# Lakonik/MVEdit

Measured on AMD Instinct MI355X. Metric: multi-view denoise-steps/sec (32 views, 512^2), higher is better.
Workload: dtype f16; 1 GPU; 32-view 512x512 get_noise_pred: 64 SD-1.5 UNet forwards (64x64 latents, ctx 77x768) + CFG per step; ControlNet residuals zero; views=32, latent=64, cfg=True, parallelism=views/1

## Files before the change

mvedit_amd/csrc/attention.hip:

```cpp
#include "common.h"

#include <stdlib.h>
#include <type_traits>

namespace {

constexpr int NT = 256;

struct AttnParams {
    const void* Q; const void* K; const void* V; const void* K2; const void* V2; void* O;
    int ldq, ldk, ldv, ldk2, ldv2, ldo;
    int B, Lq, Lk, Lk2, heads;
    float scale_log2e;
    int prescaled;
    const int* skip_if;
};

template <int DP, bool KSW2> __device__ __forceinline__ int k_perm(int row, int pc) {
    if constexpr (DP == 64) return pc ^ ((row >> 1) & 7);
    else if constexpr (KSW2) return pc ^ (((row >> 3) & 1) << 1);
    else return pc ^ ((row >> 2) & 3);
}
template <int DP, bool KSW2> __device__ __forceinline__ int k_swz(int row, int chunk) {
    return row * (DP * 2) + (k_perm<DP, KSW2>(row, chunk) << 4);
}

typedef __attribute__((address_space(3))) void* lds_ptr_t;
typedef const __attribute__((address_space(1))) void* gbl_ptr_t;
typedef float f32x8 __attribute__((ext_vector_type(8)));

__device__ __attribute__((aligned(16))) unsigned int g_attn_zero_page[4] = {0u, 0u, 0u, 0u};

template <int KB2, bool VSW2> __device__ __forceinline__ int v_swz2(int row, int chunk) {
    if constexpr (KB2 == 128) return row * 256 + ((chunk ^ (row & 15) ^ (VSW2 ? (row >> 3) & 7 : 0)) << 4);
    else return row * 128 + ((chunk ^ ((row >> 1) & 7) ^ (VSW2 ? (row >> 4) & 7 : 0)) << 4);
}

template <class Tag, int D, bool SEG2, int QF = 2, int KB2X = 0, int OCC = 0, bool KSW2 = false, bool VSW2 = false>
__global__ __launch_bounds__(NT, (OCC ? OCC : (D > 80 ? 1 : 2))) void k_attention2(const AttnParams p) {
    constexpr int QB = 64 * QF;
    constexpr int DP = (D + 31) / 32 * 32;
    constexpr int KS = DP / 32;
    constexpr int DC = D / 8;
    constexpr int DVF = (D + 15) / 16;
    constexpr int KB2 = KB2X ? KB2X : (D > 64 ? 64 : 128);
    constexpr int NH = KB2 / 64;
    constexpr int CPR = DP / 8;
    constexpr int KROW = DP * 2;
    constexpr int VROW = KB2 * 2;
    constexpr int K_BYTES = KB2 * KROW;
    constexpr int V_BYTES = DVF * 16 * VROW;
    constexpr int K_INSTR = K_BYTES / 1024 / 4;
    static_assert((K_BYTES / 1024) % 4 == 0, "K tile must split evenly over 4 waves");
    constexpr int V_TASKS = (KB2 / 2) * DC;
    constexpr int V_PER_T = (V_TASKS + NT - 1) / NT;
    constexpr bool ONES = (D % 16) != 0;
    constexpr int L_G = (D % 16) / 4, L_R = (D % 16) % 4;
    typedef typename Tag::V8 V8;
    typedef typename Tag::T T;

    __shared__ __attribute__((aligned(16))) unsigned char smem[2 * K_BYTES + 2 * V_BYTES];
    unsigned char* Kbuf = smem;
    unsigned char* Vbuf = smem + 2 * K_BYTES;

    const int tid = threadIdx.x, lane = tid & 63, wid = tid >> 6;
    const int g = lane >> 4, l16 = lane & 15;

    const int q_tiles = (p.Lq + QB - 1) / QB;
    const unsigned nblk = (unsigned)(q_tiles * p.heads * p.B);
    const unsigned bid = p.skip_if ? mve_xcd_remap_halves(blockIdx.x, nblk, nblk / 2) : mve_xcd_remap(blockIdx.x, nblk);
    const int qt = bid % q_tiles;
    const int h = (bid / q_tiles) % p.heads;
    const int b = bid / (q_tiles * p.heads);
    if (mve_second_half_skipped(p.skip_if, 2 * b >= p.B)) return;
    const int Ltot = p.Lk + p.Lk2;

    const T* Qp = reinterpret_cast<const T*>(p.Q);
    const T* zero = reinterpret_cast<const T*>(g_attn_zero_page);
    const T* kb1 = reinterpret_cast<const T*>(p.K) + (size_t)b * p.Lk * p.ldk + h * D;
    const T* vb1 = reinterpret_cast<const T*>(p.V) + (size_t)b * p.Lk * p.ldv + h * D;
    const T* kb2 = SEG2 ? reinterpret_cast<const T*>(p.K2) + (size_t)b * p.Lk2 * p.ldk2 + h * D : nullptr;
    const T* vb2 = SEG2 ? reinterpret_cast<const T*>(p.V2) + (size_t)b * p.Lk2 * p.ldv2 + h * D : nullptr;
    auto k_row = [&](int j) -> const T* {
        if constexpr (SEG2) { if (j >= p.Lk) return kb2 + (size_t)(j - p.Lk) * p.ldk2; }
        return kb1 + (size_t)j * p.ldk;
    };
    auto v_row = [&](int j) -> const T* {
        if constexpr (SEG2) { if (j >= p.Lk) return vb2 + (size_t)(j - p.Lk) * p.ldv2; }
        return vb1 + (size_t)j * p.ldv;
    };

    for (int i = tid; i < 2 * V_BYTES / 16; i += NT) reinterpret_cast<u32x4*>(Vbuf)[i] = u32x4{0u, 0u, 0u, 0u};
    __syncthreads();
    if constexpr (ONES) {
        const unsigned short one = __builtin_bit_cast(unsigned short, Tag::from_f32(1.0f));
        const unsigned two = (unsigned)one | ((unsigned)one << 16);
        for (int i = tid; i < 2 * (VROW / 4); i += NT) {
            const int buf = i / (VROW / 4), wofs = i - buf * (VROW / 4);
            *reinterpret_cast<unsigned*>(Vbuf + buf * V_BYTES + D * VROW + wofs * 4) = two;
        }
    }

    V8 qf[QF][KS];
    const int q_base = qt * QB + wid * (16 * QF);
#pragma unroll
    for (int f = 0; f < QF; ++f) {
        int q = q_base + f * 16 + l16;
        q = q < p.Lq ? q : p.Lq - 1;
        const T* row = Qp + ((size_t)b * p.Lq + q) * p.ldq + h * D;
#pragma unroll
        for (int ks = 0; ks < KS; ++ks) {
            const int c = ks * 4 + g;
            u32x4 v = {0u, 0u, 0u, 0u};
            if (c < DC) v = *reinterpret_cast<const u32x4*>(row + c * 8);
            qf[f][ks] = __builtin_bit_cast(V8, v);
        }
    }

    int kd_row[K_INSTR], kd_col[K_INSTR];
#pragma unroll
    for (int i = 0; i < K_INSTR; ++i) {
        const int pos = (wid * K_INSTR + i) * 64 + lane;
        const int row = pos / CPR, pc = pos - row * CPR;
        const int c = k_perm<DP, KSW2>(row, pc);
        kd_row[i] = row;
        kd_col[i] = c < DC ? c * 8 : -1;
    }
    int vt_key[V_PER_T], vt_col[V_PER_T], vt_lds[V_PER_T];
#pragma unroll
    for (int i = 0; i < V_PER_T; ++i) {
        const int task = tid + i * NT;
        const int pair = task / DC, c = task - pair * DC;
        const int key = 2 * pair;
        const int kk = key >> 5, hh = (key >> 4) & 1, gg = (key >> 2) & 3, jj = key & 3;
        const int pos = 32 * kk + 8 * gg + 4 * hh + jj;
        vt_key[i] = task < V_TASKS ? key : -1;
        vt_col[i] = c * 8;
        vt_lds[i] = ((pos >> 3) << 16) | ((pos & 7) * 2);
    }
    int koff[KS];
#pragma unroll
    for (int ks = 0; ks < KS; ++ks) koff[ks] = k_swz<DP, KSW2>(l16, ks * 4 + g);
    constexpr bool VTAB = VSW2 && DVF * NH * 2 <= 12;
    int voff[VTAB ? 1 : NH * 2], voff2[VTAB ? DVF : 1][NH * 2];
    if constexpr (VTAB) {
#pragma unroll
        for (int i = 0; i < DVF; ++i)
#pragma unroll
            for (int s2 = 0; s2 < NH * 2; ++s2) voff2[i][s2] = v_swz2<KB2, true>(i * 16 + l16, s2 * 4 + g);
    } else {
#pragma unroll
        for (int s2 = 0; s2 < NH * 2; ++s2) voff[s2] = v_swz2<KB2, VSW2>(l16, s2 * 4 + g);
    }
    auto vx = [](int i) { return !VSW2 ? 0 : (KB2 == 128 ? ((2 * i) & 7) << 4 : (i & 7) << 4); };

    auto dma_k = [&](int t, int buf) {
        const int j0 = t * KB2;
#pragma unroll
        for (int i = 0; i < K_INSTR; ++i) {
            int j = j0 + kd_row[i];
            j = j < Ltot ? j : Ltot - 1;
            const T* src = kd_col[i] >= 0 ? k_row(j) + kd_col[i] : zero;
            __builtin_amdgcn_global_load_lds((gbl_ptr_t)src, (lds_ptr_t)(Kbuf + buf * K_BYTES + (wid * K_INSTR + i) * 1024), 16, 0, 0);
        }
    };
    u32x4 vreg[V_PER_T][2];
    auto load_v = [&](int t) {
        const int j0 = t * KB2;
#pragma unroll
        for (int i = 0; i < V_PER_T; ++i) {
            if (vt_key[i] >= 0) {
                int j = j0 + vt_key[i];
                const int ja = j < Ltot ? j : Ltot - 1, jb = j + 1 < Ltot ? j + 1 : Ltot - 1;
                vreg[i][0] = *reinterpret_cast<const u32x4*>(v_row(ja) + vt_col[i]);
                vreg[i][1] = *reinterpret_cast<const u32x4*>(v_row(jb) + vt_col[i]);
            }
        }
    };
    auto store_v = [&](int buf) {
        unsigned char* Vs = Vbuf + buf * V_BYTES;
#pragma unroll
        for (int i = 0; i < V_PER_T; ++i) {
            if (vt_key[i] >= 0) {
                const int chunk = vt_lds[i] >> 16, within = vt_lds[i] & 0xffff;
                const unsigned short* a = reinterpret_cast<const unsigned short*>(&vreg[i][0]);
                const unsigned short* bb = reinterpret_cast<const unsigned short*>(&vreg[i][1]);
#pragma unroll
                for (int e = 0; e < 8; ++e)
                    *reinterpret_cast<unsigned*>(Vs + v_swz2<KB2, VSW2>(vt_col[i] + e, chunk) + within) = (unsigned)a[e] | ((unsigned)bb[e] << 16);
            }
        }
    };

    f32x4 oacc[DVF][QF];
#pragma unroll
    for (int i = 0; i < DVF; ++i)
#pragma unroll
        for (int f = 0; f < QF; ++f) oacc[i][f] = f32x4{0.f, 0.f, 0.f, 0.f};
    float m_run[QF], l_run[QF];
#pragma unroll
    for (int f = 0; f < QF; ++f) { m_run[f] = -INFINITY; l_run[f] = 0.f; }

    auto do_half = [&](const unsigned char* Ks, const unsigned char* Vs, int hf, int key0, auto masked_tag) {
        constexpr bool MASKED = decltype(masked_tag)::value;
        f32x4 s[4][QF];
#pragma unroll
        for (int kf = 0; kf < 4; ++kf)
#pragma unroll
            for (int f = 0; f < QF; ++f) s[kf][f] = f32x4{0.f, 0.f, 0.f, 0.f};
#pragma unroll
        for (int ks = 0; ks < KS; ++ks) {
#pragma unroll
            for (int kf = 0; kf < 4; ++kf) {
                const V8 ka = *reinterpret_cast<const V8*>(Ks + koff[ks] + (hf * 64 + kf * 16) * KROW);
#pragma unroll
                for (int f = 0; f < QF; ++f) s[kf][f] = Tag::mfma16(ka, qf[f][ks], s[kf][f]);
            }
        }
        if constexpr (MASKED) {
#pragma unroll
            for (int kf = 0; kf < 4; ++kf)
#pragma unroll
                for (int r = 0; r < 4; ++r)
                    if (key0 + kf * 16 + g * 4 + r >= Ltot) {
#pragma unroll
                        for (int f = 0; f < QF; ++f) s[kf][f][r] = -INFINITY;
                    }
        }
        V8 pf[QF][2];
#pragma unroll
        for (int f = 0; f < QF; ++f) {
            float mx = -INFINITY;
#pragma unroll
            for (int kf = 0; kf < 4; ++kf)
#pragma unroll
                for (int r = 0; r < 4; ++r) mx = fmaxf(mx, s[kf][f][r]);
            mx = mve_max_xor32(mve_max_xor16(mx));
            const float mxs = mx * p.scale_log2e;
            if (__any(mxs > m_run[f])) {
                const float m_new = fmaxf(m_run[f], mxs);
                const float alpha = __builtin_amdgcn_exp2f(m_run[f] - m_new);
                m_run[f] = m_new;
                if constexpr (!ONES) l_run[f] *= alpha;
#pragma unroll
                for (int i = 0; i < DVF; ++i)
#pragma unroll
                    for (int r = 0; r < 4; ++r) oacc[i][f][r] *= alpha;
            }
            const float mr = m_run[f];
            float psum = 0.f;
#pragma unroll
            for (int kk = 0; kk < 2; ++kk) {
                f32x8 e;
                {
                    typedef float f32x2 __attribute__((ext_vector_type(2)));
                    const f32x2 sc2 = {p.scale_log2e, p.scale_log2e}, mr2 = {mr, mr};
                    const f32x4 a4 = s[2 * kk][f], b4 = s[2 * kk + 1][f];
                    const f32x2 t0 = __builtin_elementwise_fma(f32x2{a4[0], a4[1]}, sc2, -mr2);
                    const f32x2 t1 = __builtin_elementwise_fma(f32x2{a4[2], a4[3]}, sc2, -mr2);
                    const f32x2 t2 = __builtin_elementwise_fma(f32x2{b4[0], b4[1]}, sc2, -mr2);
                    const f32x2 t3 = __builtin_elementwise_fma(f32x2{b4[2], b4[3]}, sc2, -mr2);
                    e[0] = __builtin_amdgcn_exp2f(t0[0]); e[1] = __builtin_amdgcn_exp2f(t0[1]);
                    e[2] = __builtin_amdgcn_exp2f(t1[0]); e[3] = __builtin_amdgcn_exp2f(t1[1]);
                    e[4] = __builtin_amdgcn_exp2f(t2[0]); e[5] = __builtin_amdgcn_exp2f(t2[1]);
                    e[6] = __builtin_amdgcn_exp2f(t3[0]); e[7] = __builtin_amdgcn_exp2f(t3[1]);
                }
                if constexpr (!ONES) {
#pragma unroll
                    for (int r = 0; r < 8; ++r) psum += e[r];
                }
                pf[f][kk] = __builtin_convertvector(e, V8);
            }
            if constexpr (!ONES) l_run[f] += psum;
        }
#pragma unroll
        for (int kk = 0; kk < 2; ++kk) {
#pragma unroll
            for (int i = 0; i < DVF; ++i) {
                V8 va;
                if constexpr (VTAB) va = *reinterpret_cast<const V8*>(Vs + voff2[i][hf * 2 + kk]);
                else {
                    int a = voff[hf * 2 + kk];
                    if constexpr (VSW2) { if (vx(i)) asm volatile("v_xor_b32 %0, %1, %0" : "+v"(a) : "s"(vx(i))); }
                    va = *reinterpret_cast<const V8*>(Vs + a + i * 16 * VROW);
                }
#pragma unroll
                for (int f = 0; f < QF; ++f) oacc[i][f] = Tag::mfma16(va, pf[f][kk], oacc[i][f]);
            }
        }
    };

    const int n_tiles = (Ltot + KB2 - 1) / KB2;
    dma_k(0, 0);
    load_v(0);
    __syncthreads();
    store_v(0);
    __syncthreads();

    for (int t = 0; t < n_tiles; ++t) {
        const int cur = t & 1;
        if (t + 1 < n_tiles) { dma_k(t + 1, cur ^ 1); load_v(t + 1); }
        const unsigned char* Ks = Kbuf + cur * K_BYTES;
        const unsigned char* Vs = Vbuf + cur * V_BYTES;
#pragma unroll
        for (int hf = 0; hf < NH; ++hf) {
            const int key0 = t * KB2 + hf * 64;
            if (key0 + 64 <= Ltot) {
                do_half(Ks, Vs, hf, key0, std::false_type{});
            } else if (key0 < Ltot) {
                do_half(Ks, Vs, hf, key0, std::true_type{});
            }
        }
        if (t + 1 < n_tiles) store_v(cur ^ 1);
        __syncthreads();
    }

    typedef T T4 __attribute__((ext_vector_type(4)));
#pragma unroll
    for (int f = 0; f < QF; ++f) {
        float l;
        if constexpr (ONES) {
            l = __shfl(oacc[DVF - 1][f][L_R], L_G * 16 + l16, 64);
        } else {
            l = l_run[f];
            l += __shfl_xor(l, 16, 64);
            l += __shfl_xor(l, 32, 64);
        }
        const float inv = 1.0f / l;
        const int q = q_base + f * 16 + l16;
        if (q < p.Lq) {
            T* orow = reinterpret_cast<T*>(p.O) + ((size_t)b * p.Lq + q) * p.ldo + h * D;
#pragma unroll
            for (int i = 0; i < DVF; ++i) {
                const int dv = i * 16 + g * 4;
                if (dv < D) {
                    T4 pk;
#pragma unroll
                    for (int r = 0; r < 4; ++r) pk[r] = Tag::from_f32(oacc[i][f][r] * inv);
                    *reinterpret_cast<T4*>(orow + dv) = pk;
                }
            }
        }
    }
}

__device__ __attribute__((aligned(16))) unsigned short g_attn_ones_f16[8] = {0x3C00u, 0, 0, 0, 0, 0, 0, 0};
__device__ __attribute__((aligned(16))) unsigned short g_attn_ones_bf16[8] = {0x3F80u, 0, 0, 0, 0, 0, 0, 0};

__device__ unsigned long long g_attn_prof[4] = {0ull, 0ull, 0ull, 0ull};

typedef short s16x4 __attribute__((ext_vector_type(4)));
typedef short s16x8 __attribute__((ext_vector_type(8)));
typedef float f32x2 __attribute__((ext_vector_type(2)));

__device__ __forceinline__ void attn_dma16(const void* gsrc, unsigned lds_dst) {
    unsigned keep;
    asm volatile("s_mov_b32 %0, m0\n\ts_mov_b32 m0, %2\n\ts_nop 0\n\tglobal_load_lds_dwordx4 %1, off\n\ts_mov_b32 m0, %0"
                 : "=&s"(keep) : "v"(gsrc), "s"(lds_dst) : "memory");
}

template <class Tag, bool SEG2, int NW, int NST, int WPS, bool PRE, bool PIPE, int ABL = 0>
__global__ __launch_bounds__(64 * NW, WPS) void k_attention3(const AttnParams p) {
    constexpr int D = 40, KB = 64, QB = 32 * NW;
    constexpr int K_ROW = 80, V_ROW = 96;
    constexpr int K_BYTES = KB * K_ROW, V_BYTES = KB * V_ROW, STAGE = K_BYTES + V_BYTES;
    constexpr int N_DMA = STAGE / 1024, K_DMA = K_BYTES / 1024, DMA_PER_WAVE = (N_DMA + NW - 1) / NW;
    static_assert(STAGE % 1024 == 0 && K_BYTES % 1024 == 0, "stage must split into whole LDS-DMA instructions");
    static_assert(NST >= 2 && NST <= 4, "2 to 4 LDS stages");
    typedef typename Tag::V8 V8;
    typedef typename Tag::T T;
    typedef T T2 __attribute__((ext_vector_type(2)));
    typedef T T4 __attribute__((ext_vector_type(4)));

    __shared__ __attribute__((aligned(16))) unsigned char smem[NST * STAGE];

    const int tid = threadIdx.x, lane = tid & 63, wid = tid >> 6;
    const int l32 = lane & 31, hi = lane >> 5, l16 = lane & 15, g = lane >> 4;
    unsigned long long prof_t0 = 0, prof_r0 = 0;
    if constexpr ((ABL & 1024) != 0) asm volatile("s_memtime %0\n\ts_memrealtime %1\n\ts_waitcnt lgkmcnt(0)" : "=s"(prof_t0), "=s"(prof_r0) :: "memory");

    const int q_tiles = (p.Lq + QB - 1) / QB;
    const unsigned nblk = (unsigned)(q_tiles * p.heads * p.B);
    const unsigned bid = p.skip_if ? mve_xcd_remap_halves(blockIdx.x, nblk, nblk / 2) : mve_xcd_remap(blockIdx.x, nblk);
    const int qt = bid % q_tiles;
    const int h = (bid / q_tiles) % p.heads;
    const int b = bid / (q_tiles * p.heads);
    if (mve_second_half_skipped(p.skip_if, 2 * b >= p.B)) return;
    const int Ltot = p.Lk + p.Lk2;

    const T* kb1 = reinterpret_cast<const T*>(p.K) + (size_t)b * p.Lk * p.ldk + h * D;
    const T* vb1 = reinterpret_cast<const T*>(p.V) + (size_t)b * p.Lk * p.ldv + h * D;
    const T* kb2 = SEG2 ? reinterpret_cast<const T*>(p.K2) + (size_t)b * p.Lk2 * p.ldk2 + h * D : nullptr;
    const T* vb2 = SEG2 ? reinterpret_cast<const T*>(p.V2) + (size_t)b * p.Lk2 * p.ldv2 + h * D : nullptr;
    const T* ones = reinterpret_cast<const T*>(std::is_same<T, f16>::value ? g_attn_ones_f16 : g_attn_ones_bf16);
    auto k_row = [&](int j) -> const T* {
        if constexpr (SEG2) { if (j >= p.Lk) return kb2 + (size_t)(j - p.Lk) * p.ldk2; }
        return kb1 + (size_t)j * p.ldk;
    };
    auto v_row = [&](int j) -> const T* {
        if constexpr (SEG2) { if (j >= p.Lk) return vb2 + (size_t)(j - p.Lk) * p.ldv2; }
        return vb1 + (size_t)j * p.ldv;
    };

    const int q_base = qt * QB + wid * 32;
    V8 qf[3];
    {
        int q = q_base + l32;
        q = q < p.Lq ? q : p.Lq - 1;
        const T* row = reinterpret_cast<const T*>(p.Q) + ((size_t)b * p.Lq + q) * p.ldq + h * D;
        qf[0] = __builtin_bit_cast(V8, *reinterpret_cast<const u32x4*>(row + 8 * hi));
        qf[1] = __builtin_bit_cast(V8, *reinterpret_cast<const u32x4*>(row + 16 + 8 * hi));
        u32x4 t = {0u, 0u, 0u, 0u};
        if (hi == 0) t = *reinterpret_cast<const u32x4*>(row + 32);
        qf[2] = __builtin_bit_cast(V8, t);
    }

    const int wv = __builtin_amdgcn_readfirstlane(wid);
    const unsigned smem_base = (unsigned)(uintptr_t)(lds_ptr_t)smem;
    int d_key[DMA_PER_WAVE], d_col[DMA_PER_WAVE];
    const T* d_src[DMA_PER_WAVE];
    int d_ld[DMA_PER_WAVE];
#pragma unroll
    for (int i = 0; i < DMA_PER_WAVE; ++i) {
        const int inst = wv + NW * i;
        const int o = inst * 1024 + lane * 16;
        if (inst < K_DMA) {
            const int c = o >> 4;
            d_key[i] = c / 5; d_col[i] = (c - d_key[i] * 5) * 8;
            d_ld[i] = p.ldk;
            d_src[i] = kb1 + (size_t)d_key[i] * p.ldk + d_col[i];
        } else {
            const int c = (o - K_BYTES) >> 4;
            const int r = c / 6, col = c - r * 6;
            d_key[i] = (r & ~12) | ((r & 4) << 1) | ((r & 8) >> 1);
            d_col[i] = col < 5 ? col * 8 : -1;
            d_ld[i] = col < 5 ? p.ldv : 0;
            d_src[i] = col < 5 ? vb1 + (size_t)d_key[i] * p.ldv + d_col[i] : ones;
        }
    }
    auto dma_fast = [&](int stage_off) {
#pragma unroll
        for (int i = 0; i < DMA_PER_WAVE; ++i) {
            const int inst = wv + NW * i;
            if (inst < N_DMA) {
                attn_dma16(d_src[i], smem_base + stage_off + inst * 1024);
                d_src[i] += (size_t)KB * d_ld[i];
            }
        }
    };
    auto dma_any = [&](int t, int stage_off) {
        const int j0 = t * KB;
#pragma unroll
        for (int i = 0; i < DMA_PER_WAVE; ++i) {
            const int inst = wv + NW * i;
            if (inst < N_DMA) {
                int j = j0 + d_key[i];
                j = j < Ltot ? j : Ltot - 1;
                const T* src = inst < K_DMA ? k_row(j) + d_col[i] : (d_col[i] >= 0 ? v_row(j) + d_col[i] : ones);
                attn_dma16(src, smem_base + stage_off + inst * 1024);
            }
        }
    };
    const int n_tiles = (Ltot + KB - 1) / KB, n_full = Ltot / KB;
    auto dma = [&](int t, int stage_off) {
        if constexpr ((ABL & 4) != 0) return;
        if constexpr (SEG2) dma_any(t, stage_off);
        else { if (t < n_full) dma_fast(stage_off); else dma_any(t, stage_off); }
    };
    const int n_mine = (N_DMA - wv + NW - 1) / NW;

    const int k_off01 = l32 * K_ROW + hi * 16;
    const int k_off2 = l32 * K_ROW + 64;
    const int v_off = K_BYTES + (lane >> 2) * V_ROW + (lane & 3) * 8;

    f32x4 oacc[3][2];
#pragma unroll
    for (int i = 0; i < 3; ++i)
#pragma unroll
        for (int f = 0; f < 2; ++f) oacc[i][f] = f32x4{0.f, 0.f, 0.f, 0.f};
    float m_run = PRE ? 0.f : -INFINITY;
    const float sc = p.scale_log2e;

    f32x16 negm;
#pragma unroll
    for (int r = 0; r < 16; ++r) negm[r] = 0.f;

    struct S2 { f32x16 a, b; };
    struct PB { unsigned w[2][2][4]; };

    auto qk = [&](const unsigned char* St) -> S2 {
        f32x16 zero16;
#pragma unroll
        for (int r = 0; r < 16; ++r) zero16[r] = 0.f;
        S2 s;
#pragma unroll
        for (int st = 0; st < 3; ++st) {
            const int o = st < 2 ? k_off01 + 32 * st : k_off2;
            V8 ka, kb_;
            if constexpr ((ABL & 128) != 0) { ka = qf[st]; kb_ = qf[(st + 1) % 3]; }
            else { ka = *reinterpret_cast<const V8*>(St + o); kb_ = *reinterpret_cast<const V8*>(St + o + 32 * K_ROW); }
            if constexpr ((ABL & 32) != 0) {
                asm volatile("" :: "v"(ka), "v"(kb_));
                if (st == 0) { s.a = negm; s.b = negm; }
                continue;
            }
            if (PRE && st == 0) {
                if constexpr (std::is_same<T, f16>::value) {
                    asm volatile("v_mfma_f32_32x32x16_f16 %0, %1, %2, %3" : "=&v"(s.a) : "v"(ka), "v"(qf[0]), "v"(negm));
                    asm volatile("v_mfma_f32_32x32x16_f16 %0, %1, %2, %3" : "=&v"(s.b) : "v"(kb_), "v"(qf[0]), "v"(negm));
                } else {
                    asm volatile("v_mfma_f32_32x32x16_bf16 %0, %1, %2, %3" : "=&v"(s.a) : "v"(ka), "v"(qf[0]), "v"(negm));
                    asm volatile("v_mfma_f32_32x32x16_bf16 %0, %1, %2, %3" : "=&v"(s.b) : "v"(kb_), "v"(qf[0]), "v"(negm));
                }
            } else {
                s.a = Tag::mfma32(ka, qf[st], st == 0 ? zero16 : s.a);
                s.b = Tag::mfma32(kb_, qf[st], st == 0 ? zero16 : s.b);
            }
        }
        return s;
    };

    auto softmax_max = [&](S2& s, int key0, auto masked_tag, bool first) {
        constexpr bool MASKED = decltype(masked_tag)::value;
        if constexpr (MASKED) {
#pragma unroll
            for (int r = 0; r < 16; ++r) {
                if (key0 + (r & 3) + 8 * (r >> 2) + 4 * hi >= Ltot) s.a[r] = -INFINITY;
                if (key0 + 32 + (r & 3) + 8 * (r >> 2) + 4 * hi >= Ltot) s.b[r] = -INFINITY;
            }
        }
        float mx = fmaxf(s.a[0], s.b[0]);
        if constexpr ((ABL & 16) == 0) {
#pragma unroll
            for (int r = 1; r < 16; ++r) mx = fmaxf(fmaxf(mx, s.a[r]), s.b[r]);
            mx = mve_max_xor32(mx);
        }
        float a0 = 1.f, a1 = 1.f;
        bool rescale = false;
        if constexpr (PRE) {
            if (__builtin_expect(first || __any(mx > 0.f), 0)) {
                const float delta = first ? mx : fmaxf(mx, 0.f);
                m_run += delta;
#pragma unroll
                for (int r = 0; r < 16; ++r) { s.a[r] -= delta; s.b[r] -= delta; negm[r] = -m_run; }
                if (!first) {
                    const float alpha = __builtin_amdgcn_exp2f(-delta);
                    const auto ar = __builtin_amdgcn_permlane16_swap(__float_as_uint(alpha), __float_as_uint(alpha), false, false);
                    a0 = __uint_as_float(ar[0]); a1 = __uint_as_float(ar[1]);
                    rescale = true;
                }
            }
        } else {
            const float mxs = mx * sc;
            if (__builtin_expect(__any(mxs > m_run), 0)) {
                const float m_new = fmaxf(m_run, mxs);
                const float alpha = __builtin_amdgcn_exp2f(m_run - m_new);
                m_run = m_new;
                const auto ar = __builtin_amdgcn_permlane16_swap(__float_as_uint(alpha), __float_as_uint(alpha), false, false);
                a0 = __uint_as_float(ar[0]); a1 = __uint_as_float(ar[1]);
                rescale = true;
            }
        }
        if (rescale) {
#pragma unroll
            for (int i = 0; i < 3; ++i)
#pragma unroll
                for (int r = 0; r < 4; ++r) { oacc[i][0][r] *= a0; oacc[i][1][r] *= a1; }
        }
    };

    auto softmax_exp = [&](const S2& s) -> PB {
        const float nm = -m_run;
        PB pb;
#pragma unroll
        for (int kb = 0; kb < 2; ++kb) {
            const f32x16& sk = kb ? s.b : s.a;
            unsigned pk[8];
#pragma unroll
            for (int r2 = 0; r2 < 8; ++r2) {
                float e0, e1;
                if constexpr (PRE && (ABL & 8) != 0) {
                    e0 = sk[2 * r2]; e1 = sk[2 * r2 + 1];
                } else if constexpr (PRE) {
                    e0 = __builtin_amdgcn_exp2f(sk[2 * r2]);
                    e1 = __builtin_amdgcn_exp2f(sk[2 * r2 + 1]);
                } else {
                    e0 = __builtin_amdgcn_exp2f(__builtin_fmaf(sk[2 * r2], sc, nm));
                    e1 = __builtin_amdgcn_exp2f(__builtin_fmaf(sk[2 * r2 + 1], sc, nm));
                }
                pk[r2] = __builtin_bit_cast(unsigned, __builtin_convertvector(f32x2{e0, e1}, T2));
            }
#pragma unroll
            for (int v = 0; v < 4; ++v) {
                const int ai = v < 2 ? v : v + 2;
                if constexpr ((ABL & 512) != 0) { pb.w[kb][0][v] = pk[ai]; pb.w[kb][1][v] = pk[ai + 2]; continue; }
                const auto r = __builtin_amdgcn_permlane16_swap(pk[ai], pk[ai + 2], false, false);
                pb.w[kb][0][v] = r[0];
                pb.w[kb][1][v] = r[1];
            }
        }
        return pb;
    };

    auto pv = [&](const unsigned char* St, const PB& pb) {
#pragma unroll
        for (int kb = 0; kb < 2; ++kb) {
            s16x4 lo[3], up[3];
            const unsigned va0 = (unsigned)(uintptr_t)(lds_ptr_t)(St + v_off + kb * 32 * V_ROW);
            if constexpr ((ABL & 256) != 0) {
#pragma unroll
                for (int i = 0; i < 3; ++i) { lo[i] = __builtin_bit_cast(s16x4, u32x2{pb.w[kb][0][i], va0}); up[i] = __builtin_bit_cast(s16x4, u32x2{va0, pb.w[kb][1][i]}); }
            } else {
                typedef __attribute__((address_space(3))) s16x4* lp;
#pragma unroll
                for (int i = 0; i < 3; ++i) {
                    lo[i] = __builtin_amdgcn_ds_read_tr16_b64_v4i16((lp)(lds_ptr_t)(St + v_off + kb * 32 * V_ROW + 32 * i));
                    up[i] = __builtin_amdgcn_ds_read_tr16_b64_v4i16((lp)(lds_ptr_t)(St + v_off + kb * 32 * V_ROW + 32 * i + 16 * V_ROW));
                }
            }
#pragma unroll
            for (int i = 0; i < 3; ++i) {
                const V8 va = __builtin_bit_cast(V8, __builtin_shufflevector(lo[i], up[i], 0, 1, 2, 3, 4, 5, 6, 7));
#pragma unroll
                for (int f = 0; f < 2; ++f) {
                    const u32x4 pw = {pb.w[kb][f][0], pb.w[kb][f][1], pb.w[kb][f][2], pb.w[kb][f][3]};
                    if constexpr ((ABL & 64) != 0) { asm volatile("" : "+v"(oacc[i][f]) : "v"(va), "v"(pw)); continue; }
                    oacc[i][f] = Tag::mfma16(va, __builtin_bit_cast(V8, pw), oacc[i][f]);
                }
            }
        }
    };

    auto wait_sync = [&](int keep) {
        if constexpr ((ABL & 3) == 3) { asm volatile("s_waitcnt lgkmcnt(0)" ::: "memory"); return; }
        else if constexpr ((ABL & 1) != 0) { asm volatile("s_waitcnt vmcnt(0)\n\ts_waitcnt lgkmcnt(0)" ::: "memory"); return; }
        else if constexpr ((ABL & 2) != 0) { asm volatile("s_waitcnt lgkmcnt(0)\n\ts_barrier" ::: "memory"); return; }
        if (keep >= 3) asm volatile("s_waitcnt vmcnt(3)\n\ts_waitcnt lgkmcnt(0)\n\ts_barrier" ::: "memory");
        else if (keep == 2) asm volatile("s_waitcnt vmcnt(2)\n\ts_waitcnt lgkmcnt(0)\n\ts_barrier" ::: "memory");
        else if (keep == 1) asm volatile("s_waitcnt vmcnt(1)\n\ts_waitcnt lgkmcnt(0)\n\ts_barrier" ::: "memory");
        else asm volatile("s_waitcnt vmcnt(0)\n\ts_waitcnt lgkmcnt(0)\n\ts_barrier" ::: "memory");
    };
    auto next_stage = [&](int off) { return off + STAGE == NST * STAGE ? 0 : off + STAGE; };

    if constexpr (!PIPE) {
        constexpr int PD = NST - 1;
        static_assert(DMA_PER_WAVE * (PD - 1) <= 3, "wait_sync covers at most three outstanding instructions");
#pragma unroll
        for (int i = 0; i < PD; ++i)
            if (i < n_tiles) dma(i, i * STAGE);
        asm volatile("" : "+v"(qf[0]), "+v"(qf[1]), "+v"(qf[2]));
        wait_sync(n_mine * ((n_tiles < PD ? n_tiles : PD) - 1));
        int cur = 0, nxt = PD * STAGE;
        for (int t = 0; t < n_full; ++t) {
            if (t + PD < n_tiles) dma(t + PD, nxt);
            S2 s = qk(smem + cur);
            softmax_max(s, t * KB, std::false_type{}, t == 0);
            const PB pb = softmax_exp(s);
            pv(smem + cur, pb);
            const int last_issued = t + PD < n_tiles ? t + PD : n_tiles - 1;
            wait_sync(last_issued > t + 1 ? n_mine * (last_issued - (t + 1)) : 0);
            nxt = cur;
            cur = next_stage(cur);
        }
        if (n_full < n_tiles) {
            S2 s = qk(smem + cur);
            softmax_max(s, n_full * KB, std::true_type{}, n_full == 0);
            const PB pb = softmax_exp(s);
            pv(smem + cur, pb);
        }
    } else {
        static_assert(NST >= 3, "the pipelined loop needs the next tile's K resident");
        constexpr int PD = NST - 1;
        static_assert(DMA_PER_WAVE * (PD - 2) <= 3, "wait_sync covers at most three outstanding instructions");
#pragma unroll
        for (int i = 0; i < PD; ++i)
            if (i < n_tiles) dma(i, i * STAGE);
        asm volatile("" : "+v"(qf[0]), "+v"(qf[1]), "+v"(qf[2]));
        {
            const int issued = n_tiles < PD ? n_tiles : PD;
            wait_sync(issued > 2 ? n_mine * (issued - 2) : 0);
        }
        int cur = 0, nx1 = STAGE, nxt = (PD % NST) * STAGE;
        S2 sA = qk(smem), sB;
        const int n_main = n_tiles - 1;
        auto step = [&](S2& sc_, S2& sn_, int t) {
            if (t + PD < n_tiles) dma(t + PD, nxt);
            softmax_max(sc_, t * KB, std::false_type{}, t == 0);
            sn_ = qk(smem + nx1);
            const PB pb = softmax_exp(sc_);
            pv(smem + cur, pb);
            const int last_issued = t + PD < n_tiles ? t + PD : n_tiles - 1;
            wait_sync(last_issued > t + 2 ? n_mine * (last_issued - (t + 2)) : 0);
            nxt = cur; cur = nx1; nx1 = next_stage(nx1);
        };
        int t = 0;
        for (; t + 2 <= n_main; t += 2) { step(sA, sB, t); step(sB, sA, t + 1); }
        if (t < n_main) { step(sA, sB, t); sA = sB; ++t; }
        if (n_full < n_tiles) softmax_max(sA, t * KB, std::true_type{}, t == 0);
        else softmax_max(sA, t * KB, std::false_type{}, t == 0);
        const PB pb = softmax_exp(sA);
        pv(smem + cur, pb);
    }

#pragma unroll
    for (int f = 0; f < 2; ++f) {
        const float l = __shfl(oacc[2][f][0], 32 + l16, 64);
        const float inv = 1.0f / l;
        const int q = q_base + f * 16 + l16;
        if (q < p.Lq) {
            T* orow = reinterpret_cast<T*>(p.O) + ((size_t)b * p.Lq + q) * p.ldo + h * D;
#pragma unroll
            for (int i = 0; i < 3; ++i) {
                const int dv = i * 16 + g * 4;
                if (dv < D) {
                    T4 o4;
#pragma unroll
                    for (int r = 0; r < 4; ++r) o4[r] = Tag::from_f32(oacc[i][f][r] * inv);
                    *reinterpret_cast<T4*>(orow + dv) = o4;
                }
            }
        }
    }
    if constexpr ((ABL & 1024) != 0) {
        unsigned long long t1, r1;
        asm volatile("s_memtime %0\n\ts_memrealtime %1\n\ts_waitcnt lgkmcnt(0)" : "=s"(t1), "=s"(r1) :: "memory");
        if (lane == 0 && (blockIdx.x & 63) == 5) {
            atomicAdd(&g_attn_prof[0], t1 - prof_t0);
            atomicAdd(&g_attn_prof[1], r1 - prof_r0);
            atomicAdd(&g_attn_prof[2], 1ull);
        }
    }
}

int g_attn_variant = 9;
int g_attn_ablate = 0;

template <class Tag, int D>
int launch(const AttnParams& p, hipStream_t s) {
    if constexpr (D == 40) {
        if (g_attn_variant >= 8 && g_attn_variant <= 15) {
            const int var = g_attn_variant;
            const bool w8 = var == 9 || var == 11 || var >= 14;
            const unsigned grid3 = (unsigned)(((p.Lq + (w8 ? 255 : 127)) / (w8 ? 256 : 128)) * p.heads * p.B);
#define MVE_A3P(SEG, NW_, NST_, WPS_, PRE_, PIPE_) k_attention3<Tag, SEG, NW_, NST_, WPS_, PRE_, PIPE_><<<grid3, 64 * NW_, 0, s>>>(p)
#define MVE_A3(NW_, NST_, WPS_, PIPE_) do { \
                if (p.Lk2 > 0) { if (p.prescaled && !PIPE_) MVE_A3P(true, NW_, NST_, WPS_, (!PIPE_), PIPE_); else MVE_A3P(true, NW_, NST_, WPS_, false, PIPE_); } \
                else { if (p.prescaled && !PIPE_) MVE_A3P(false, NW_, NST_, WPS_, (!PIPE_), PIPE_); else MVE_A3P(false, NW_, NST_, WPS_, false, PIPE_); } } while (0)
#ifdef MVE_ATTN_LAB
            if (g_attn_ablate != 0) {
                if constexpr (std::is_same<Tag, F16Tag>::value) {
                    if (p.Lk2 == 0 && p.prescaled) {
                        const unsigned grid9 = (unsigned)(((p.Lq + 255) / 256) * p.heads * p.B);
                        bool hit = true;
                        switch (g_attn_ablate) {
#define MVE_ABL(A) case A: k_attention3<Tag, false, 8, 2, 4, true, false, (A) | 1024><<<grid9, 512, 0, s>>>(p); break;
                            MVE_ABL(2048) MVE_ABL(1) MVE_ABL(3) MVE_ABL(7) MVE_ABL(8) MVE_ABL(16) MVE_ABL(24) MVE_ABL(32) MVE_ABL(64) MVE_ABL(96) MVE_ABL(128) MVE_ABL(256)
                            MVE_ABL(384) MVE_ABL(512) MVE_ABL(536) MVE_ABL(927) MVE_ABL(480) MVE_ABL(1023)
#undef MVE_ABL
                            default: hit = false;
                        }
                        if (hit) { MVE_LAUNCH_CHECK(); return MVE_OK; }
                    }
                }
            }
#endif
            switch (var) {
                case 8: MVE_A3(4, 2, 4, false); break;
                case 9: MVE_A3(8, 2, 4, false); break;
                case 10: MVE_A3(4, 3, 4, false); break;
                case 11: MVE_A3(8, 3, 4, false); break;
                case 12: MVE_A3(4, 3, 3, true); break;
                case 13: MVE_A3(4, 4, 3, true); break;
                case 14: MVE_A3(8, 3, 2, true); break;
                default: MVE_A3(8, 4, 2, true); break;
            }
#undef MVE_A3P
#undef MVE_A3
            MVE_LAUNCH_CHECK();
            return MVE_OK;
        }
        if (g_attn_variant == 1 && p.Lk2 == 0) {
            const unsigned grid1 = (unsigned)(((p.Lq + 63) / 64) * p.heads * p.B);
            k_attention2<Tag, D, false, 1, 64, 3><<<grid1, NT, 0, s>>>(p);
            MVE_LAUNCH_CHECK();
            return MVE_OK;
        }
    }
    constexpr int QB = 128;
    const unsigned grid = (unsigned)(((p.Lq + QB - 1) / QB) * p.heads * p.B);
    const int var = g_attn_variant >= 8 ? ((D == 80 || D == 160) ? 6 : 4) : g_attn_variant;
    if constexpr (D == 80 || D == 160) {
        if ((var == 2 || var == 6) && p.Lk2 == 0) {
            if (var == 6) k_attention2<Tag, D, false, 2, 0, 0, true, true><<<grid, NT, 0, s>>>(p);
            else k_attention2<Tag, D, false, 2, 0, 0, true><<<grid, NT, 0, s>>>(p);
            MVE_LAUNCH_CHECK();
            return MVE_OK;
        }
    }
    if ((var == 4 || var == 6) && p.Lk2 == 0) {
        k_attention2<Tag, D, false, 2, 0, 0, false, true><<<grid, NT, 0, s>>>(p);
        MVE_LAUNCH_CHECK();
        return MVE_OK;
    }
    if (p.Lk2 > 0) k_attention2<Tag, D, true><<<grid, NT, 0, s>>>(p);
    else k_attention2<Tag, D, false><<<grid, NT, 0, s>>>(p);
    MVE_LAUNCH_CHECK();
    return MVE_OK;
}

template <class Tag>
int dispatch_d(const AttnParams& p, int d, hipStream_t s) {
    switch (d) {
        case 40: return launch<Tag, 40>(p, s);
        case 64: return launch<Tag, 64>(p, s);
        case 80: return launch<Tag, 80>(p, s);
        case 160: return launch<Tag, 160>(p, s);
        default:
            mve_set_error("attention: unsupported head dim %d (supported: 40, 64, 80, 160)", d);
            return MVE_ERR_ARG;
    }
}

}

extern "C" int mve_attention_profile(unsigned long long* out4) {
    MVE_CHECK(out4, MVE_ERR_ARG, "attention_profile: null pointer");
#ifndef MVE_ATTN_LAB
    mve_set_error("attention_profile: the timing-only ablation kernels are compiled into development builds only (MVE_ATTN_LAB=1 python -m mvedit_amd.build)");
    return MVE_ERR_STATE;
#endif
    MVE_HIP(hipDeviceSynchronize());
    MVE_HIP(hipMemcpyFromSymbol(out4, HIP_SYMBOL(g_attn_prof), 4 * sizeof(unsigned long long)));
    const unsigned long long z[4] = {0ull, 0ull, 0ull, 0ull};
    MVE_HIP(hipMemcpyToSymbol(HIP_SYMBOL(g_attn_prof), z, sizeof(z)));
    return MVE_OK;
}

extern "C" int mve_attention_tune(int variant) {
    const int old = g_attn_variant | (g_attn_ablate << 8);
#ifndef MVE_ATTN_LAB
    if (variant >= 256) { mve_set_error("attention_tune: ablation bits (8-19) need a development build (MVE_ATTN_LAB=1)"); return MVE_ERR_ARG; }
#endif
    if (variant >= 0) { g_attn_variant = variant & 255; g_attn_ablate = (variant >> 8) & 4095; }
    return old;
}

static int attention_entry(int dtype, const void* Q, int ldq, const void* K, int ldk, const void* V, int ldv,
                           const void* K2, int ldk2, const void* V2, int ldv2, void* O, int ldo, int B, int Lq,
                           int Lk, int Lk2, int heads, int head_dim, float scale, int prescaled, void* stream) {
    if (B == 0 || Lq == 0) return MVE_OK;
    MVE_CHECK(Q && K && V && O, MVE_ERR_ARG, "attention: null pointer");
    MVE_CHECK(Lk > 0 && Lk2 >= 0 && heads > 0, MVE_ERR_ARG, "attention: bad sizes Lk=%d Lk2=%d heads=%d", Lk, Lk2, heads);
    MVE_CHECK(Lk2 == 0 || (K2 && V2), MVE_ERR_ARG, "attention: second KV segment has null pointers");
    MVE_CHECK(ldq % 8 == 0 && ldk % 8 == 0 && ldv % 8 == 0 && ldo % 4 == 0 && (Lk2 == 0 || (ldk2 % 8 == 0 && ldv2 % 8 == 0)),
              MVE_ERR_ARG, "attention: leading dimensions must be multiples of 8");
    AttnParams p;
    p.Q = Q; p.K = K; p.V = V; p.K2 = K2; p.V2 = V2; p.O = O;
    p.ldq = ldq; p.ldk = ldk; p.ldv = ldv; p.ldk2 = ldk2; p.ldv2 = ldv2; p.ldo = ldo;
    p.B = B; p.Lq = Lq; p.Lk = Lk; p.Lk2 = Lk2; p.heads = heads;
    p.scale_log2e = prescaled ? 1.0f : scale * 1.4426950408889634f;
    p.prescaled = prescaled;
    p.skip_if = mve_skip_second_half();
    MVE_CHECK(!p.skip_if || B % 2 == 0, MVE_ERR_ARG, "attention: the second-half predicate needs an even batch (B=%d)", B);
    if (dtype == MVE_F16) return dispatch_d<F16Tag>(p, head_dim, (hipStream_t)stream);
    if (dtype == MVE_BF16) return dispatch_d<BF16Tag>(p, head_dim, (hipStream_t)stream);
    mve_set_error("attention: unsupported dtype %d", dtype);
    return MVE_ERR_ARG;
}

extern "C" int mve_attention(int dtype, const void* Q, int ldq, const void* K, int ldk, const void* V, int ldv,
                             const void* K2, int ldk2, const void* V2, int ldv2, void* O, int ldo, int B, int Lq,
                             int Lk, int Lk2, int heads, int head_dim, float scale, void* stream) {
    return attention_entry(dtype, Q, ldq, K, ldk, V, ldv, K2, ldk2, V2, ldv2, O, ldo, B, Lq, Lk, Lk2, heads, head_dim, scale, 0, stream);
}

extern "C" int mve_attention_prescaled(int dtype, const void* Q, int ldq, const void* K, int ldk, const void* V, int ldv,
                                       const void* K2, int ldk2, const void* V2, int ldv2, void* O, int ldo, int B, int Lq,
                                       int Lk, int Lk2, int heads, int head_dim, void* stream) {
    return attention_entry(dtype, Q, ldq, K, ldk, V, ldv, K2, ldk2, V2, ldv2, O, ldo, B, Lq, Lk, Lk2, heads, head_dim, 1.0f, 1, stream);
}
```

Before: 16.15 denoise-steps/s.

## Stream V tiles straight to LDS and read them with transposing LDS loads

Adds a VTR path to the attention kernel for head dims 64/80/160. V tiles are copied row-major into LDS with global_load_lds DMA, and ds_read_tr16_b64 transposes them during the read, replacing the register load, scalar scatter and zero-fill of V. Synchronisation now waits on vmcnt before each barrier. The path is on by default for the SD UNet head sizes, including the SEG2 case. It removes VGPR staging and LDS write traffic, but adds a new swizzle pattern that may cause bank conflicts or layout bugs.

```diff
diff --git a/mvedit_amd/csrc/attention.hip b/mvedit_amd/csrc/attention.hip
--- a/mvedit_amd/csrc/attention.hip
+++ b/mvedit_amd/csrc/attention.hip
@@ -28,15 +28,28 @@
 typedef __attribute__((address_space(3))) void* lds_ptr_t;
 typedef const __attribute__((address_space(1))) void* gbl_ptr_t;
 typedef float f32x8 __attribute__((ext_vector_type(8)));
+typedef short s16x4 __attribute__((ext_vector_type(4)));
 
 __device__ __attribute__((aligned(16))) unsigned int g_attn_zero_page[4] = {0u, 0u, 0u, 0u};
+
+__device__ __forceinline__ void attn_dma16(const void* gsrc, unsigned lds_dst) {
+    unsigned keep;
+    asm volatile("s_mov_b32 %0, m0\n\ts_mov_b32 m0, %2\n\ts_nop 0\n\tglobal_load_lds_dwordx4 %1, off\n\ts_mov_b32 m0, %0"
+                 : "=&s"(keep) : "v"(gsrc), "s"(lds_dst) : "memory");
+}
 
 template <int KB2, bool VSW2> __device__ __forceinline__ int v_swz2(int row, int chunk) {
     if constexpr (KB2 == 128) return row * 256 + ((chunk ^ (row & 15) ^ (VSW2 ? (row >> 3) & 7 : 0)) << 4);
     else return row * 128 + ((chunk ^ ((row >> 1) & 7) ^ (VSW2 ? (row >> 4) & 7 : 0)) << 4);
 }
 
-template <class Tag, int D, bool SEG2, int QF = 2, int KB2X = 0, int OCC = 0, bool KSW2 = false, bool VSW2 = false>
+template <int D> __device__ __forceinline__ int vtr_perm(int row, int chunk) {
+    if constexpr (D == 64) return chunk ^ (((row >> 1) & 3) << 1);
+    else if constexpr (D == 160) return chunk ^ (((row >> 2) & 1) << 1);
+    else return chunk;
+}
+
+template <class Tag, int D, bool SEG2, int QF = 2, int KB2X = 0, int OCC = 0, bool KSW2 = false, bool VSW2 = false, bool VTR = false>
 __global__ __launch_bounds__(NT, (OCC ? OCC : (D > 80 ? 1 : 2))) void k_attention2(const AttnParams p) {
     constexpr int QB = 64 * QF;
     constexpr int DP = (D + 31) / 32 * 32;
@@ -53,7 +66,13 @@
     constexpr int K_INSTR = K_BYTES / 1024 / 4;
     static_assert((K_BYTES / 1024) % 4 == 0, "K tile must split evenly over 4 waves");
     constexpr int V_TASKS = (KB2 / 2) * DC;
-    constexpr int V_PER_T = (V_TASKS + NT - 1) / NT;
+    constexpr int V_PER_T = VTR ? 1 : (V_TASKS + NT - 1) / NT;
+    static_assert(!VTR || ((D == 64 || D == 80 || D == 160) && !VSW2), "transposed-read V path: d = 64 / 80 / 160");
+    constexpr int VTROW = D * 2;
+    constexpr int V_DMA = V_BYTES / 1024;
+    constexpr int V_INSTR = (V_DMA + 3) / 4;
+    constexpr int NV = D == 64 ? 4 : (D == 160 ? 2 : 1);
+    static_assert(!VTR || (V_BYTES == KB2 * VTROW && V_BYTES % 1024 == 0), "row-major V tile must fill the V^T image");
     constexpr bool ONES = (D % 16) != 0;
     constexpr int L_G = (D % 16) / 4, L_R = (D % 16) % 4;
     typedef typename Tag::V8 V8;
@@ -90,8 +109,10 @@
         return vb1 + (size_t)j * p.ldv;
     };
 
-    for (int i = tid; i < 2 * V_BYTES / 16; i += NT) reinterpret_cast<u32x4*>(Vbuf)[i] = u32x4{0u, 0u, 0u, 0u};
-    __syncthreads();
+    if constexpr (!VTR) {
+        for (int i = tid; i < 2 * V_BYTES / 16; i += NT) reinterpret_cast<u32x4*>(Vbuf)[i] = u32x4{0u, 0u, 0u, 0u};
+        __syncthreads();
+    }
     if constexpr (ONES) {
         const unsigned short one = __builtin_bit_cast(unsigned short, Tag::from_f32(1.0f));
         const unsigned two = (unsigned)one | ((unsigned)one << 16);
@@ -152,6 +173,38 @@
 #pragma unroll
         for (int s2 = 0; s2 < NH * 2; ++s2) voff[s2] = v_swz2<KB2, VSW2>(l16, s2 * 4 + g);
     }
+    const int wv = __builtin_amdgcn_readfirstlane(wid);
+    const unsigned smem_base = (unsigned)(uintptr_t)(lds_ptr_t)smem;
+    auto dma_sync = [&]() {
+        if constexpr (VTR) asm volatile("s_waitcnt vmcnt(0)" ::: "memory");
+        __syncthreads();
+    };
+    int vd_row[VTR ? V_INSTR : 1], vd_col[VTR ? V_INSTR : 1], vtr_off[VTR ? NV : 1];
+    if constexpr (VTR) {
+#pragma unroll
+        for (int i = 0; i < V_INSTR; ++i) {
+            const int pos = (wv + 4 * i) * 64 + lane;
+            const int row = pos / DC, pc = pos - row * DC;
+            vd_row[i] = row;
+            vd_col[i] = vtr_perm<D>(row, pc) * 8;
+        }
+#pragma unroll
+        for (int n = 0; n < NV; ++n) vtr_off[n] = (lane >> 2) * VTROW + (vtr_perm<D>(lane >> 2, 2 * n) << 4) + (lane & 3) * 8;
+    }
+    auto dma_v = [&](int t, int buf) {
+        if constexpr (VTR) {
+            const int j0 = t * KB2;
+#pragma unroll
+            for (int i = 0; i < V_INSTR; ++i) {
+                const int inst = wv + 4 * i;
+                if (inst < V_DMA) {
+                    const int j = j0 + vd_row[i];
+                    const T* src = j < Ltot ? v_row(j) + vd_col[i] : zero;
+                    attn_dma16(src, smem_base + 2 * K_BYTES + buf * V_BYTES + inst * 1024);
+                }
+            }
+        }
+    };
     auto vx = [](int i) { return !VSW2 ? 0 : (KB2 == 128 ? ((2 * i) & 7) << 4 : (i & 7) << 4); };
 
     auto dma_k = [&](int t, int buf) {
@@ -161,11 +214,13 @@
             int j = j0 + kd_row[i];
             j = j < Ltot ? j : Ltot - 1;
             const T* src = kd_col[i] >= 0 ? k_row(j) + kd_col[i] : zero;
-            __builtin_amdgcn_global_load_lds((gbl_ptr_t)src, (lds_ptr_t)(Kbuf + buf * K_BYTES + (wid * K_INSTR + i) * 1024), 16, 0, 0);
+            if constexpr (VTR) attn_dma16(src, smem_base + buf * K_BYTES + (wv * K_INSTR + i) * 1024);
+            else __builtin_amdgcn_global_load_lds((gbl_ptr_t)src, (lds_ptr_t)(Kbuf + buf * K_BYTES + (wid * K_INSTR + i) * 1024), 16, 0, 0);
         }
     };
     u32x4 vreg[V_PER_T][2];
     auto load_v = [&](int t) {
+        if constexpr (VTR) { dma_v(t, t & 1); return; }
         const int j0 = t * KB2;
 #pragma unroll
         for (int i = 0; i < V_PER_T; ++i) {
@@ -178,6 +233,7 @@
         }
     };
     auto store_v = [&](int buf) {
+        if constexpr (VTR) return;
         unsigned char* Vs = Vbuf + buf * V_BYTES;
 #pragma unroll
         for (int i = 0; i < V_PER_T; ++i) {
@@ -278,7 +334,13 @@
 #pragma unroll
             for (int i = 0; i < DVF; ++i) {
                 V8 va;
-                if constexpr (VTAB) va = *reinterpret_cast<const V8*>(Vs + voff2[i][hf * 2 + kk]);
+                if constexpr (VTR) {
+                    typedef __attribute__((address_space(3))) s16x4* lp;
+                    const unsigned char* a = Vs + vtr_off[i % NV] + ((2 * i) & ~(2 * NV - 1)) * 16 + (hf * 2 + kk) * 32 * VTROW;
+                    const s16x4 lo = __builtin_amdgcn_ds_read_tr16_b64_v4i16((lp)(lds_ptr_t)a);
+                    const s16x4 up = __builtin_amdgcn_ds_read_tr16_b64_v4i16((lp)(lds_ptr_t)(a + 16 * VTROW));
+                    va = __builtin_bit_cast(V8, __builtin_shufflevector(lo, up, 0, 1, 2, 3, 4, 5, 6, 7));
+                } else if constexpr (VTAB) va = *reinterpret_cast<const V8*>(Vs + voff2[i][hf * 2 + kk]);
                 else {
                     int a = voff[hf * 2 + kk];
                     if constexpr (VSW2) { if (vx(i)) asm volatile("v_xor_b32 %0, %1, %0" : "+v"(a) : "s"(vx(i))); }
@@ -293,9 +355,15 @@
     const int n_tiles = (Ltot + KB2 - 1) / KB2;
     dma_k(0, 0);
     load_v(0);
-    __syncthreads();
+    if constexpr (!VTR) __syncthreads();
     store_v(0);
-    __syncthreads();
+    if constexpr (VTR) {
+#pragma unroll
+        for (int f = 0; f < QF; ++f)
+#pragma unroll
+            for (int ks = 0; ks < KS; ++ks) asm volatile("" : "+v"(qf[f][ks]));
+    }
+    dma_sync();
 
     for (int t = 0; t < n_tiles; ++t) {
         const int cur = t & 1;
@@ -312,7 +380,7 @@
             }
         }
         if (t + 1 < n_tiles) store_v(cur ^ 1);
-        __syncthreads();
+        dma_sync();
     }
 
     typedef T T4 __attribute__((ext_vector_type(4)));
@@ -349,15 +417,8 @@
 
 __device__ unsigned long long g_attn_prof[4] = {0ull, 0ull, 0ull, 0ull};
 
-typedef short s16x4 __attribute__((ext_vector_type(4)));
 typedef short s16x8 __attribute__((ext_vector_type(8)));
 typedef float f32x2 __attribute__((ext_vector_type(2)));
-
-__device__ __forceinline__ void attn_dma16(const void* gsrc, unsigned lds_dst) {
-    unsigned keep;
-    asm volatile("s_mov_b32 %0, m0\n\ts_mov_b32 m0, %2\n\ts_nop 0\n\tglobal_load_lds_dwordx4 %1, off\n\ts_mov_b32 m0, %0"
-                 : "=&s"(keep) : "v"(gsrc), "s"(lds_dst) : "memory");
-}
 
 template <class Tag, bool SEG2, int NW, int NST, int WPS, bool PRE, bool PIPE, int ABL = 0>
 __global__ __launch_bounds__(64 * NW, WPS) void k_attention3(const AttnParams p) {
@@ -738,8 +799,8 @@
 template <class Tag, int D>
 int launch(const AttnParams& p, hipStream_t s) {
     if constexpr (D == 40) {
-        if (g_attn_variant >= 8 && g_attn_variant <= 15) {
-            const int var = g_attn_variant;
+        if (g_attn_variant >= 8 && g_attn_variant <= 16) {
+            const int var = g_attn_variant == 16 ? 9 : g_attn_variant;
             const bool w8 = var == 9 || var == 11 || var >= 14;
             const unsigned grid3 = (unsigned)(((p.Lq + (w8 ? 255 : 127)) / (w8 ? 256 : 128)) * p.heads * p.B);
 #define MVE_A3P(SEG, NW_, NST_, WPS_, PRE_, PIPE_) k_attention3<Tag, SEG, NW_, NST_, WPS_, PRE_, PIPE_><<<grid3, 64 * NW_, 0, s>>>(p)
@@ -789,6 +850,26 @@
     constexpr int QB = 128;
     const unsigned grid = (unsigned)(((p.Lq + QB - 1) / QB) * p.heads * p.B);
     const int var = g_attn_variant >= 8 ? ((D == 80 || D == 160) ? 6 : 4) : g_attn_variant;
+    if constexpr (D == 64 || D == 80 || D == 160) {
+        constexpr bool VTR_DEFAULT = true;
+        if (g_attn_variant == 16 || (g_attn_variant >= 8 && VTR_DEFAULT)) {
+            constexpr bool KS = D != 64;
+            static const bool said = [] {
+                if (getenv("MVE_DEBUG")) {
+                    int nb_old = -1, nb_new = -1;
+                    (void)hipOccupancyMaxActiveBlocksPerMultiprocessor(&nb_old, reinterpret_cast<const void*>(&k_attention2<Tag, D, false, 2, 0, 0, KS, true>), NT, 0);
+                    (void)hipOccupancyMaxActiveBlocksPerMultiprocessor(&nb_new, reinterpret_cast<const void*>(&k_attention2<Tag, D, false, 2, 0, 0, KS, false, true>), NT, 0);
+                    fprintf(stderr, "[mve] k_attention2<%d>: %d blocks per CU by the occupancy API with the transposed-read V path, %d without\n", D, nb_new, nb_old);
+                }
+                return true;
+            }();
+            (void)said;
+            if (p.Lk2 > 0) k_attention2<Tag, D, true, 2, 0, 0, false, false, true><<<grid, NT, 0, s>>>(p);
+            else k_attention2<Tag, D, false, 2, 0, 0, KS, false, true><<<grid, NT, 0, s>>>(p);
+            MVE_LAUNCH_CHECK();
+            return MVE_OK;
+        }
+    }
     if constexpr (D == 80 || D == 160) {
         if ((var == 2 || var == 6) && p.Lk2 == 0) {
             if (var == 6) k_attention2<Tag, D, false, 2, 0, 0, true, true><<<grid, NT, 0, s>>>(p);
```

Result: no change. 16.26 denoise-steps/s, median of 6 (+0.7%).
